# FangjinhuaWang/IterMVS

Hardware: AMD Instinct MI355X
Metric: depth-maps/sec (ref-views/s) at 5-view 640x512, 4 iters (higher is better)
Workload: dtype f32; 1 GPU; BASELINE cfg 2 (= cfg 1 on 1xMI355X): 1 ref + 4 src views, 640x512, 4 GRU iterations, test mode, random-init weights, 1 ref view(s) per step and GPU; views=5, height=512, width=640, batch_per_gpu=1, streams_per_gpu=1, feature_dtype=fp32, launch=one hipGraph per depth map, parallelism=ref-view sharding x1, no collective, projection=device_fp64, conv_arithmetic=bf16x3, side_branch=False

## Files before the change

include/itermvs_hip.h:

```cpp
#ifndef ITERMVS_HIP_H
#define ITERMVS_HIP_H

#include <stdint.h>

#ifdef __cplusplus
extern "C" {
#endif

#if defined(__GNUC__) || defined(__clang__)
#pragma GCC visibility push(default)
#endif

#define ITERMVS_ABI_VERSION 20
#define ITERMVS_MAX_SRC 16
#define ITERMVS_MAX_HYP 8
#define ITERMVS_GROUPS 8
#define ITERMVS_PROB_BINS 256
#define ITERMVS_WINDOW_RADIUS 4

typedef enum itermvs_status {
    ITERMVS_OK = 0,
    ITERMVS_ERR_NULL = -1,
    ITERMVS_ERR_DIMS = -2,
    ITERMVS_ERR_CHANNELS = -3,
// ... 246 lines not shown
    ITERMVS_WALK_PLAIN = 2,
    ITERMVS_WALK_STRIDED_LEAD = 3
} itermvs_walk_kind;

typedef struct itermvs_persistent_plan_t {
    int32_t grid, banded, run, run_extra;
} itermvs_persistent_plan_t;

int itermvs_persistent_plan(int64_t tiles, int32_t resident, int32_t round8, int32_t kind, itermvs_persistent_plan_t* out);
int itermvs_tile_walk_owner(const itermvs_persistent_plan_t* plan, int64_t tiles, int32_t kind, int32_t lead, int32_t* owner, int32_t* order);

int itermvs_corrnet(const float* x, int64_t x_sn, const float* const* weights, const int32_t* seg_end, int32_t n_seg,
                    int32_t M, int32_t H, int32_t W, float* out, int64_t out_sn, float* out2, int64_t out2_sn, void* stream);
int itermvs_corrnet_bf16x3(const float* x, int64_t x_sn, const float* const* weights, const int32_t* seg_end, int32_t n_seg,
                           int32_t M, int32_t H, int32_t W, float* out, int64_t out_sn, float* out2, int64_t out2_sn, void* stream);


int itermvs_stem(const float* x, int64_t x_sn, int32_t M, int32_t H, int32_t W, const float* w0, const float* w1,
                 float* y, float* sc, int64_t out_sn, int32_t out_layout, void* stream);
int itermvs_stem_compose(const float* x, int64_t x_sn, int32_t M, int32_t H, int32_t W, const float* w0, const float* w1,
                         float* y, float* sc, int64_t out_sn, int32_t out_layout, const float* mats, int32_t n_sets, int32_t V, float* proj_out,
                         int32_t* nan_flag, const float* depth_min, const float* depth_max, int32_t Bd, float* inv_min,
                         float* inv_max, void* stream);



int itermvs_fuse_depth(const float* depth_ref, const float* conf_ref, const float* const* depth_src,
                       const float* mats, int32_t S, int32_t H, int32_t W, double geo_pixel_thres,
                       float geo_depth_thres, float photo_thres, int32_t geo_mask_thres, double* depth_avg,
                       uint8_t* photo_mask, uint8_t* geo_mask, uint8_t* final_mask, int32_t* geo_sum,
                       void* stream);

int itermvs_fuse_depth_claim(const float* depth_ref, const float* conf_ref, const float* const* depth_src,
                             const float* mats, int32_t S, int32_t H, int32_t W, double geo_pixel_thres,
                             float geo_depth_thres, float photo_thres, int32_t geo_mask_thres, double* depth_avg,
                             uint8_t* photo_mask, uint8_t* geo_mask, uint8_t* final_mask, int32_t* geo_sum,
                             const uint8_t* claimed_ref, uint8_t* const* claimed_src, void* stream);

int itermvs_fuse_points_workspace_bytes(int32_t H, int32_t W);
int itermvs_fuse_points(const double* depth_avg, const uint8_t* final_mask, const uint8_t* photo_mask,
                        const uint8_t* geo_mask, const float* cam, const uint8_t* rgb, int32_t H, int32_t W,
                        uint8_t* records, int64_t capacity, uint64_t* cursor, int64_t* view_counts, int32_t view,
                        uint32_t* workspace, void* stream);

int itermvs_fuse_points_normals(const double* depth_avg, const uint8_t* final_mask, const uint8_t* photo_mask,
                                const uint8_t* geo_mask, const float* cam, const uint8_t* rgb, int32_t H, int32_t W,
// ... 93 lines not shown
```

itermvs_amd/_lib.py:

```python
from __future__ import annotations

import ctypes as C
import os
from typing import Optional

MAX_SRC = 16
MAX_HYP = 8
GROUPS = 8
F32, F16, BF16 = 0, 1, 2
GT_DTU, GT_BLENDEDMVS = 0, 1
ABI_VERSION = 20

_HERE = os.path.dirname(os.path.abspath(__file__))
LIB_PATH = os.path.join(_HERE, "libitermvs_hip.so")

c_float_p = C.POINTER(C.c_float)


class FMap(C.Structure):
    _fields_ = [("data", C.c_void_p), ("sb", C.c_int64), ("sc", C.c_int64), ("sy", C.c_int64),
                ("sx", C.c_int64), ("C", C.c_int32), ("H", C.c_int32), ("W", C.c_int32), ("dtype", C.c_int32)]


class LevelSrc(C.Structure):
# ... 119 lines not shown
                                      C.c_void_p]),
    "itermvs_conv2d": (C.c_int, [C.POINTER(ConvParams), C.c_void_p]),
    "itermvs_conv2d_plan": (C.c_int, [C.POINTER(ConvParams), C.POINTER(ConvPlan)]),
    "itermvs_persistent_plan": (C.c_int, [C.c_int64, C.c_int32, C.c_int32, C.c_int32, C.POINTER(PersistentPlan)]),
    "itermvs_tile_walk_owner": (C.c_int, [C.POINTER(PersistentPlan), C.c_int64, C.c_int32, C.c_int32, C.c_void_p, C.c_void_p]),
    "itermvs_corrnet": (C.c_int, [C.c_void_p, C.c_int64, C.POINTER(C.c_void_p), C.POINTER(C.c_int32), C.c_int32, C.c_int32, C.c_int32,
                                  C.c_int32, C.c_void_p, C.c_int64, C.c_void_p, C.c_int64, C.c_void_p]),
    "itermvs_corrnet_bf16x3": (C.c_int, [C.c_void_p, C.c_int64, C.POINTER(C.c_void_p), C.POINTER(C.c_int32), C.c_int32, C.c_int32, C.c_int32,
                                  C.c_int32, C.c_void_p, C.c_int64, C.c_void_p, C.c_int64, C.c_void_p]),
    "itermvs_res_chain16": (C.c_int, [C.c_void_p, C.c_int64, C.c_void_p, C.c_int64, C.c_int32, C.c_int32, C.c_int32, C.c_int32,
                                      C.POINTER(C.c_void_p), C.POINTER(C.c_void_p), C.c_void_p, C.c_int64, C.c_void_p]),
    "itermvs_down_conv": (C.c_int, [C.c_void_p, C.c_int64, C.c_int32, C.c_int32, C.c_int32, C.c_int32, C.c_void_p, C.c_void_p, C.c_int32,
                                    C.c_void_p, C.c_int64, C.c_void_p, C.c_int64, C.c_void_p]),
    "itermvs_lateral_conv3x3": (C.c_int, [C.c_void_p, C.c_int64, C.c_int32, C.c_void_p, C.c_int64, C.c_int32, C.c_int32, C.c_int32,
                                          C.c_void_p, C.c_void_p, C.c_void_p, C.c_void_p, C.c_int32, C.c_void_p, C.c_int64, C.c_int32,
                                          C.c_void_p, C.c_void_p]),
    "itermvs_gru_conv": (C.c_int, [C.c_void_p, C.c_int64, C.c_int32, C.c_int32, C.c_int32, C.c_int32, C.c_void_p, C.c_void_p, C.c_void_p,
                                   C.c_int64, C.c_void_p, C.c_int64, C.c_void_p, C.c_int64, C.c_void_p, C.c_int64, C.c_void_p]),
    "itermvs_stem": (C.c_int, [C.c_void_p, C.c_int64, C.c_int32, C.c_int32, C.c_int32, C.c_void_p, C.c_void_p, C.c_void_p, C.c_void_p,
                               C.c_int64, C.c_int32, C.c_void_p]),
    "itermvs_stem_compose": (C.c_int, [C.c_void_p, C.c_int64, C.c_int32, C.c_int32, C.c_int32, C.c_void_p, C.c_void_p, C.c_void_p, C.c_void_p,
                                       C.c_int64, C.c_int32, C.c_void_p, C.c_int32, C.c_int32, C.c_void_p, C.c_void_p, C.c_void_p, C.c_void_p,
                                       C.c_int32, C.c_void_p, C.c_void_p, C.c_void_p]),
    "itermvs_image_pyramid": (C.c_int, [C.c_void_p] + [C.c_int32] * 5 + [C.c_void_p] * 5),
    "itermvs_resize_rgb8": (C.c_int, [C.c_void_p] + [C.c_int32] * 5 + [C.c_void_p, C.c_void_p, C.c_int32, C.c_void_p, C.c_void_p,
                                                                 C.c_int32, C.c_void_p, C.c_void_p]),
    "itermvs_undistort_rgb8": (C.c_int, [C.c_void_p, C.c_int32, C.c_int32, C.c_int32, C.POINTER(C.c_double), C.c_int32] +
                               [C.c_double] * 4 + [C.c_int32, C.c_int32, C.c_void_p, C.c_void_p, C.c_void_p]),
    "itermvs_image_pyramid_jitter": (C.c_int, [C.c_void_p] + [C.c_int32] * 5 + [C.c_void_p] * 7),
    "itermvs_gt_pyramid": (C.c_int, [C.c_void_p] * 3 + [C.c_int32] * 6 + [C.c_void_p] * 9),
    "itermvs_bn_workspace_floats": (C.c_int, [C.c_int32, C.c_int32, C.c_int32]),
    "itermvs_bn_train_forward": (C.c_int, [C.c_void_p, C.c_void_p, C.c_int32, C.c_int32, C.c_int32, C.c_void_p, C.c_void_p,
                                           C.c_float, C.c_float, C.c_int32, C.c_void_p, C.c_void_p, C.c_void_p, C.c_void_p,
                                           C.c_void_p, C.c_void_p]),
    "itermvs_bn_train_backward": (C.c_int, [C.c_void_p, C.c_void_p, C.c_void_p, C.c_int32, C.c_int32, C.c_int32, C.c_void_p,
                                            C.c_void_p, C.c_void_p, C.c_void_p, C.c_int32, C.c_void_p, C.c_void_p, C.c_void_p,
                                            C.c_void_p]),
    "itermvs_profile_enable": (C.c_int, [C.c_int32]),
    "itermvs_profile_set_mask": (C.c_int, [C.c_int32]),
    "itermvs_fuse_depth": (C.c_int, [C.c_void_p, C.c_void_p, C.c_void_p, C.c_void_p, C.c_int32, C.c_int32, C.c_int32, C.c_double,
                                     C.c_float, C.c_float, C.c_int32, C.c_void_p, C.c_void_p, C.c_void_p, C.c_void_p, C.c_void_p,
                                     C.c_void_p]),
    "itermvs_fuse_depth_claim": (C.c_int, [C.c_void_p, C.c_void_p, C.c_void_p, C.c_void_p, C.c_int32, C.c_int32, C.c_int32,
                                           C.c_double, C.c_float, C.c_float, C.c_int32, C.c_void_p, C.c_void_p, C.c_void_p,
                                           C.c_void_p, C.c_void_p, C.c_void_p, C.c_void_p, C.c_void_p]),
    "itermvs_fuse_points_workspace_bytes": (C.c_int, [C.c_int32, C.c_int32]),
# ... 78 lines not shown
```

itermvs_amd/csrc/stem.hip:

```cpp
#include "common.hpp"
#include "compose.hpp"
#include "tile_walk.hpp"
#include <cstdlib>

namespace itermvs {

using f32x4 = __attribute__((ext_vector_type(4))) float;
typedef __attribute__((address_space(4))) float ConstF;

constexpr int kStTW = 32;
constexpr int kStThreads = 256;
constexpr int kStIP = 68;
constexpr int kStFP = 66;

struct StemArgs {
    const float* x;
    const float* w0;
    const float* w1;
    float* y;
    float* sc;
    int64_t x_sn, out_sn;
    int M, H, W, H2, W2, tiles_x, tiles_y;
    int out_c4;
};

using f32x2 = __attribute__((ext_vector_type(2))) float;

template <int kStTH>
struct StemPatch {
    static constexpr int IR = 2 * kStTH + 3, ROWS = 3 * IR, PER = (ROWS + 3) / 4;
    float v[PER], vt[PER];
    unsigned rowok;
    bool c0ok, c1ok;
    __device__ __forceinline__ void fetch(const StemArgs& a, int tile, int wave, int lane) {
        int t = tile;
        const int tx = t % a.tiles_x; t /= a.tiles_x;
        const int ty = t % a.tiles_y;
        const int n = t / a.tiles_y;
        const int iy0 = 2 * ty * kStTH - 2, ix0 = 2 * tx * kStTW - 2;
        const float* __restrict__ xp = a.x + (int64_t)n * a.x_sn;
        const int plane = a.H * a.W;
        const int gx0 = ix0 + lane, gx1 = ix0 + 64 + (lane < 3 ? lane : 2);
        c0ok = gx0 >= 0 && gx0 < a.W;
        c1ok = lane < 3 && gx1 < a.W;
        const int cx0 = min(max(gx0, 0), a.W - 1), cx1 = min(gx1, a.W - 1);
        rowok = 0;
#pragma unroll
        for (int i = 0; i < PER; ++i) {
            const int row = min(wave + 4 * i, ROWS - 1);
            const int ci = row / IR, r = row - ci * IR;
            const int gy = iy0 + r;
            rowok |= (wave + 4 * i < ROWS && gy >= 0 && gy < a.H) ? 1u << i : 0u;
            const float* __restrict__ rp = xp + ci * plane + min(max(gy, 0), a.H - 1) * a.W;
            v[i] = rp[cx0];
            vt[i] = rp[cx1];
        }
    }
    __device__ __forceinline__ void commit(float* __restrict__ IMG, int wave, int lane) const {
#pragma unroll
        for (int i = 0; i < PER; ++i) {
            const int row = wave + 4 * i;
            if (row < ROWS) {
                const bool rok = rowok >> i & 1u;
                IMG[row * kStIP + lane] = rok && c0ok ? v[i] : 0.0f;
                if (lane < 3) IMG[row * kStIP + 64 + lane] = rok && c1ok ? vt[i] : 0.0f;
            }
        }
    }
};

template <int kStTH>
__global__ __launch_bounds__(kStThreads) void stem_kernel(StemArgs a, int tiles, int n_comp, ComposeArgs comp) {
    if ((int)blockIdx.x < n_comp) {
        compose_proj_body(comp, (int)blockIdx.x * kStThreads + (int)threadIdx.x);
        return;
    }
    const TileWalk walk = tile_walk_strided(tiles, blockIdx.x, gridDim.x, n_comp, (int)gridDim.x - n_comp >= 8);
    const int tile0 = walk.w, tstep = walk.wstep, tend = walk.wend;

    constexpr int kStIR = 2 * kStTH + 3, kStFR = 2 * kStTH + 1;
    constexpr int kStFPL = kStFR * kStFP + 1;
    static_assert(kStFPL % 2 == 1, "f0 plane stride must be odd");
    __shared__ float IMG[3 * kStIR * kStIP];
    __shared__ float F0[8 * kStFPL];
    const int tid = threadIdx.x, lane = tid & 63;
    const int wave = __builtin_amdgcn_readfirstlane(tid >> 6);
    const int q = lane >> 4, l16 = lane & 15;

    StemPatch<kStTH> patch;
    if (tile0 < tend) patch.fetch(a, tile0, wave, lane);

    float aw[36];
#pragma unroll
    for (int i = 0; i < 18; ++i) {
        aw[2 * i] = a.w1[(i * 4 + q) * 32 + l16];
        aw[2 * i + 1] = a.w1[(i * 4 + q) * 32 + 16 + l16];
    }
    const float* __restrict__ bias = a.w1 + 9 * 2 * 4 * 32;
    float bv[2][4];
#pragma unroll
    for (int mb = 0; mb < 2; ++mb)
#pragma unroll
        for (int r = 0; r < 4; ++r) bv[mb][r] = bias[mb * 16 + q * 4 + r];
    const int oplane = a.H2 * a.W2;

#pragma unroll 1
    for (int tile = tile0; tile < tend; tile += tstep) {
        int t = tile;
        const int tx = t % a.tiles_x; t /= a.tiles_x;
        const int ty = t % a.tiles_y;
        const int n = t / a.tiles_y;
        const int oy0 = ty * kStTH, ox0 = tx * kStTW;
        const int iy0 = 2 * oy0 - 2, ix0 = 2 * ox0 - 2;

        patch.commit(IMG, wave, lane);
        __syncthreads();
        if (tile + tstep < tend) patch.fetch(a, tile + tstep, wave, lane);

        constexpr int ITEMS = kStFR * 64 + kStFR, ROUNDS = (ITEMS + kStThreads - 1) / kStThreads;
#pragma unroll 1
        for (int it = 0; it < ROUNDS; ++it) {
            int opaque = 0;
            asm volatile("" : "+s"(opaque));
            const ConstF* w0 = (const ConstF*)(uintptr_t)a.w0 + __builtin_amdgcn_readfirstlane(opaque);
            const int rr = wave + 4 * it;
            const bool tail = rr >= kStFR;
            const int r = tail ? lane : rr, c = tail ? 64 : lane;
            if (tail && (rr > kStFR || lane >= kStFR)) continue;
            float v[27];
            const float* __restrict__ ip = IMG + r * kStIP + c;
#pragma unroll
            for (int ci = 0; ci < 3; ++ci)
#pragma unroll
                for (int ky = 0; ky < 3; ++ky)
#pragma unroll
                    for (int kx = 0; kx < 3; ++kx) v[(ci * 3 + ky) * 3 + kx] = ip[(ci * kStIR + ky) * kStIP + kx];
            const int gy = iy0 + 1 + r, gx = ix0 + 1 + c;
            const bool inside = gy >= 0 && gy < a.H && gx >= 0 && gx < a.W;
            f32x2 acc[4];
#pragma unroll
            for (int c2 = 0; c2 < 4; ++c2) acc[c2] = f32x2{w0[216 + 2 * c2], w0[217 + 2 * c2]};
#pragma unroll
            for (int k = 0; k < 27; ++k)
#pragma unroll
                for (int c2 = 0; c2 < 4; ++c2)
                    acc[c2] = __builtin_elementwise_fma(f32x2{w0[k * 8 + 2 * c2], w0[k * 8 + 2 * c2 + 1]}, f32x2{v[k], v[k]}, acc[c2]);
            float* __restrict__ fp = F0 + r * kStFP + c;
#pragma unroll
            for (int co = 0; co < 8; ++co) fp[co * kStFPL] = inside ? fmaxf(acc[co >> 1][co & 1], 0.0f) : 0.0f;
        }
        __syncthreads();

#pragma unroll
        for (int gi = 0; gi < kStTH / 2; ++gi) {
            const int g = wave + 4 * gi;
            const int oy = g >> 1, oxl = (g & 1) * 16 + l16;
            f32x4 acc[2];
#pragma unroll
            for (int mb = 0; mb < 2; ++mb) acc[mb] = f32x4{bv[mb][0], bv[mb][1], bv[mb][2], bv[mb][3]};
            const float* __restrict__ bp = F0 + q * kStFPL + 2 * oy * kStFP + 2 * oxl;
#pragma unroll
            for (int tap = 0; tap < 9; ++tap) {
                const int ky = tap / 3, kx = tap - ky * 3;
#pragma unroll
                for (int ks = 0; ks < 2; ++ks) {
                    const float b = bp[ks * 4 * kStFPL + ky * kStFP + kx];
                    acc[0] = __builtin_amdgcn_mfma_f32_16x16x4f32(aw[(tap * 2 + ks) * 2], b, acc[0], 0, 0, 0);
                    acc[1] = __builtin_amdgcn_mfma_f32_16x16x4f32(aw[(tap * 2 + ks) * 2 + 1], b, acc[1], 0, 0, 0);
                }
            }
            const int gy = oy0 + oy, gx = ox0 + oxl;
            if (gy < a.H2 && gx < a.W2) {
                if (a.out_c4) {
                    const int64_t o = (int64_t)n * a.out_sn + ((int64_t)q * oplane + gy * a.W2 + gx) * 4;
                    *reinterpret_cast<f32x4*>(a.y + o) =
                        f32x4{fmaxf(acc[0][0], 0.0f), fmaxf(acc[0][1], 0.0f), fmaxf(acc[0][2], 0.0f), fmaxf(acc[0][3], 0.0f)};
                    *reinterpret_cast<f32x4*>(a.sc + o) = acc[1];
                } else {
                    const int64_t o = (int64_t)n * a.out_sn + (int64_t)(q * 4) * oplane + gy * a.W2 + gx;
                    float* __restrict__ yo = a.y + o;
                    float* __restrict__ so = a.sc + o;
#pragma unroll
                    for (int r = 0; r < 4; ++r) {
                        yo[r * oplane] = fmaxf(acc[0][r], 0.0f);
                        so[r * oplane] = acc[1][r];
                    }
                }
            }
        }
    }
}

}

static int launch_stem(const float* x, int64_t x_sn, int32_t M, int32_t H, int32_t W, const float* w0, const float* w1,
                       float* y, float* sc, int64_t out_sn, int32_t out_layout, const itermvs::ComposeArgs* comp, void* stream) {
    using namespace itermvs;
    if (!x || !w0 || !w1 || !y || !sc) return ITERMVS_ERR_NULL;
    if (M < 0 || H < 1 || W < 1) return ITERMVS_ERR_DIMS;
    if (out_layout != 0 && out_layout != 1) return ITERMVS_ERR_LAYOUT;
    if (out_layout == 1 && (((uintptr_t)y | (uintptr_t)sc) % 16 || out_sn % 4)) return ITERMVS_ERR_ALIGN;
    ComposeArgs c{};
    int n_comp = 0;
    if (comp) {
        c = *comp;
        int ct = c.n_sets * (c.V - 1);
        if (c.inv_min && c.B > ct) ct = c.B;
        n_comp = (ct + kStThreads - 1) / kStThreads;
    }
    if (M == 0 && n_comp == 0) return ITERMVS_OK;
    StemArgs a;
    a.x = x; a.w0 = w0; a.w1 = w1; a.y = y; a.sc = sc;
    a.x_sn = x_sn; a.out_sn = out_sn; a.out_c4 = out_layout;
    a.M = M; a.H = H; a.W = W;
    a.H2 = (H - 1) / 2 + 1; a.W2 = (W - 1) / 2 + 1;
    static const int th = [] { const char* e = itermvs_tuning_env("ITERMVS_STEM_TH"); return e && atoi(e) == 4 ? 4 : 8; }();
    a.tiles_x = (a.W2 + kStTW - 1) / kStTW; a.tiles_y = (a.H2 + th - 1) / th;
    const int64_t tiles = (int64_t)M * a.tiles_x * a.tiles_y;
    static const int wg_per_cu = [] { const char* e = itermvs_tuning_env("ITERMVS_STEM_WGS"); return e ? atoi(e) : 0; }();
    PersistentPlan plan = {};
    if (tiles != 0) {
        const int rc = persistent_plan_cus(tiles, wg_per_cu > 0 ? wg_per_cu : (th == 4 ? 4 : 3), false, ITERMVS_WALK_STRIDED_LEAD, &plan);
        if (rc != ITERMVS_OK) return rc;
    }
    const unsigned grid = (unsigned)plan.grid + (unsigned)n_comp;
    if (th == 4) hipLaunchKernelGGL(stem_kernel<4>, dim3(grid), dim3(kStThreads), 0, (hipStream_t)stream, a, (int)tiles, n_comp, c);
    else hipLaunchKernelGGL(stem_kernel<8>, dim3(grid), dim3(kStThreads), 0, (hipStream_t)stream, a, (int)tiles, n_comp, c);
    return itermvs_launch_status();
}

extern "C" int itermvs_stem(const float* x, int64_t x_sn, int32_t M, int32_t H, int32_t W, const float* w0, const float* w1,
                            float* y, float* sc, int64_t out_sn, int32_t out_layout, void* stream) {
    return launch_stem(x, x_sn, M, H, W, w0, w1, y, sc, out_sn, out_layout, nullptr, stream);
}

extern "C" int itermvs_stem_compose(const float* x, int64_t x_sn, int32_t M, int32_t H, int32_t W, const float* w0, const float* w1,
                                    float* y, float* sc, int64_t out_sn, int32_t out_layout, const float* mats, int32_t n_sets, int32_t V,
                                    float* proj_out, int32_t* nan_flag, const float* depth_min, const float* depth_max, int32_t Bd,
                                    float* inv_min, float* inv_max, void* stream) {
    ITERMVS_RETURN_IF(!mats || !proj_out, ITERMVS_ERR_NULL);
    ITERMVS_RETURN_IF(inv_min && (!depth_min || !depth_max || !inv_max || Bd < 1), ITERMVS_ERR_NULL);
    ITERMVS_RETURN_IF(n_sets < 1, ITERMVS_ERR_DIMS);
    ITERMVS_RETURN_IF(V < 2 || V - 1 > ITERMVS_MAX_SRC, ITERMVS_ERR_VIEWS);
    const itermvs::ComposeArgs c{mats, proj_out, nan_flag, depth_min, depth_max, inv_min, inv_max, n_sets, V, Bd};
    return launch_stem(x, x_sn, M, H, W, w0, w1, y, sc, out_sn, out_layout, &c, stream);
}
```

itermvs_amd/engine.py:

```python
from __future__ import annotations

import gc
import itertools
import weakref
from typing import Dict, List, Mapping, Tuple

import torch

from . import ops

Tensor = torch.Tensor

INIT_SAMPLES = 32
HIDDEN = 32
_INTERVALS = {1: (-2.0, -2.0 / 3, 2.0 / 3, 2.0), 2: (-8.0, -8.0 / 3, 8.0 / 3, 8.0), 3: (-32.0, 32.0)}


def sample_offsets() -> Dict[int, Tuple[float, ...]]:
    out = {}
    for l, vals in _INTERVALS.items():
        t = torch.tensor(vals, dtype=torch.float32) * (1.0 / 256)
        out[l] = tuple(float(v) for v in t)
    return out

# ... 43 lines not shown
        self.side_branch = side_branch
        self._side = None
        self.profile_iterations = None
        self.profile_init = True
        self.pk: Dict[str, object] = {}
        self._pack_weights()

    def _pack_weights(self) -> None:
        w, pk = self.w, self.pk
        pack = lambda wt: ops.pack_conv_weight(wt) if (wt.shape[1] <= 4 or wt.shape[0] == 1) and wt.shape[2] == 3 else ops.MfmaWeight(wt, split3=self.split3)
        for n, (wt, _) in self.cbr.items():
            pk["feature_net." + n] = pack(wt)
        for k, v in w.items():
            if not k.endswith("weight") or v.dim() != 4 or ".bn." in k or k.startswith("feature_net.") and ".conv." in k:
                continue
            if k.endswith("conv3.weight") or k.endswith("conv4.weight"):
                pk[k] = ops.MfmaWeight(v, transposed=True)
            else:
                pk[k] = pack(v)
        pv = "iter_mvs.evaluation.pixel_view_weight.conv.1."
        cf = "iter_mvs.update.confidence_head.2."
        self.conf_dot = torch.cat([w[cf + "weight"].reshape(-1), w[cf + "bias"].reshape(-1)]).float().contiguous()
        self.pvw_dot = torch.cat([w[pv + "weight"].reshape(-1), w[pv + "bias"].reshape(-1)]).float().contiguous()
        self.stem_w = ops.pack_stem_weights(*self.cbr["conv1."], *self.cbr["layer1.0.conv1."], *self.cbr["layer1.0.downsample."])
        self.corrnet_w = {l: ops.pack_corrnet_weights(w, f"iter_mvs.evaluation.corr_conv1.{l - 1}.", split3=self.split3) for l in (1, 2, 3)}
        dh = "iter_mvs.update.depth_head."
        self.head_w1, self.head_w2 = ops.pack_head_weights(w[dh + "2.weight"], w[dh + "4.weight"])
        if self.split3:
            self.head_w2_fused = ops.pack_head_w2_split3(w[dh + "4.weight"])
            self.head_w0_fused = ops.pack_head_w0_split3(w[dh + "0.weight"])
        else:
            self.head_w2_fused = self.head_w2
            self.head_w0_fused = None
        self.pk_zr = ops.MfmaWeight(self.w_zr, split3=False)
        self.gru_coop = self.split3
        if self.gru_coop:
            g = "iter_mvs.update.gru."
            self.gru_zr = ops.pack_gru_conv_split3(self.w_zr)
            self.gru_q = ops.pack_gru_conv_split3(w[g + "convq.weight"])
            self.gru_bq = w[g + "convq.bias"].contiguous()
        hi, up = "iter_mvs.update.hidden_init_head.", "iter_mvs.upsample."
        self.pk_hi0, self.pk_up0 = ops.MfmaWeight(w[hi + "0.weight"], split3=False), ops.MfmaWeight(w[up + "0.weight"], split3=False)
        self.hi1, self.hi1_bias = ops.pack_conv1x1_operand(w[hi + "2.weight"], w[hi + "2.bias"])
        self.up1, _ = ops.pack_conv1x1_operand(w[up + "2.weight"])
        if self.split3:
            self.pk_hi0, self.hi1, self.hi1_bias = ops.pack_conv3x3_conv1x1_split3(w[hi + "0.weight"], w[hi + "2.weight"], w[hi + "2.bias"])
            self.pk_up0, self.up1, _ = ops.pack_conv3x3_conv1x1_split3(w[up + "0.weight"], w[up + "2.weight"])
# ... 27 lines not shown
            y = ops.conv2d(x, wt, bias, stride=2, act="relu", split=(c, "none", sc))
        return self._cbr(y, name + "conv2.", 1, "relu", add=sc)

    def feature_net(self, x: Tensor, compose=None, out: Tuple[Tensor, Tensor, Tensor, Tensor] = None) -> Dict[int, Tensor]:
        p = "feature_net."
        m, _, hh, ww = x.shape
        dev = x.device
        if out is not None:
            o1, o2, o3, self.o2_planar = out
            want = [((m, 16, hh // 2, ww // 2), self.feature_dtype), ((m, 32, hh // 4, ww // 4), self.feature_dtype),
                    ((m, 48, hh // 8, ww // 8), self.feature_dtype)]
            for t, (shape, dt) in zip((o1, o2, o3), want):
                if tuple(t.shape) != shape or t.dtype != dt or not t.is_contiguous(memory_format=torch.channels_last):
                    raise RuntimeError(f"feature_net: out level must be a dense channels-last {dt} tensor {shape}")
            p2 = self.o2_planar
            if tuple(p2.shape) != (m, 32, hh // 4, ww // 4) or p2.dtype != torch.float32 or not p2.is_contiguous():
                raise RuntimeError(f"feature_net: the planar level-2 map must be a contiguous float32 {(m, 32, hh // 4, ww // 4)}")
        else:
            cl = lambda c, s: torch.empty((m, c, hh // s, ww // s), device=dev, dtype=self.feature_dtype,
                                          memory_format=torch.channels_last)
            o1, o2, o3 = cl(16, 2), cl(32, 4), cl(48, 8)
            self.o2_planar = torch.empty((m, 32, hh // 4, ww // 4), device=dev)
        if compose is not None:
            y, sc, *self.composed = ops.stem(x, *self.stem_w, compose=compose, quads=self.split3)
        else:
            y, sc = ops.stem(x, *self.stem_w, quads=self.split3)
        if self.split3:
            names = ("layer1.0.conv2.", "layer1.1.conv1.", "layer1.1.conv2.")
            f1 = ops.res_chain16(y, sc, [self.pk[p + k] for k in names], [self.cbr[k][1] for k in names], quads=True)
        else:
            f1 = self._res(self._cbr(y, "layer1.0.conv2.", 1, "relu", add=sc), "layer1.1.", 1)
        f2 = self._res(self._res(f1, "layer2.0.", 2), "layer2.1.", 1)
        f3 = self._res(self._res(f2, "layer3.0.", 2), "layer3.1.", 1)
        self._conv(f3, p + "output3.", bias=True, channels_last_out=True, out=o3)
        mid = self._conv(f2, p + "inner2.", bias=True, ksize=1, pad=0, add=f3, add_up2=True)
        self._conv(mid, p + "output2.", bias=True, channels_last_out=True, out=o2, out2=self.o2_planar)
        if self.split3:
            ops.lateral_conv3x3(f1, mid, self.pk[p + "inner1.weight"], self.w[p + "inner1.bias"], self.pk[p + "output1.weight"],
                                self.w[p + "output1.bias"], out=o1, channels_last_out=True)
        else:
            mid = self._conv(f1, p + "inner1.", bias=True, ksize=1, pad=0, add=mid, add_up2=True)
            self._conv(mid, p + "output1.", bias=True, channels_last_out=True, out=o1)
        return {1: o1, 2: o2, 3: o3}

    def corr_nets(self, x: Tensor, levels, seg_end=(), out: Tensor = None, out2: Tensor = None) -> Tensor:
        return ops.corrnet(x, [self.corrnet_w[l] for l in levels], seg_end, out=out, out2=out2)

    def depth_head(self, hidden: Tensor) -> Tensor:
        p = "iter_mvs.update.depth_head."
# ... 541 lines not shown
```

itermvs_amd/ops.py:

```python
from __future__ import annotations

import contextlib
import ctypes as C
import os
from typing import Dict, List, NamedTuple, Optional, Sequence, Tuple

import numpy as np
import torch

from . import _lib
from ._lib import MAX_HYP, MAX_SRC, ConvParams, CorrInitParams, CorrIterParams, FMap, LevelSlots, LevelSrc, TapParams, check

Tensor = torch.Tensor


def _stream() -> int:
    return torch.cuda.current_stream().cuda_stream


def _dev(t: Tensor, name: str) -> Tensor:
    if not isinstance(t, torch.Tensor) or not t.is_cuda:
        raise RuntimeError(f"{name}: expected a CUDA/ROCm tensor - the IterMVS HIP engine has no CPU path")
    if t.dtype != torch.float32:
        raise RuntimeError(f"{name}: expected float32, got {t.dtype}")
# ... 1499 lines not shown
        for v in range(6):
            for term in (h, m_):
                ops_a.append(torch.stack([term[2 * v], term[2 * v + 1], term[2 * v], term[2 * v + 1]]))
        for v in range(6):
            ops_a.append(torch.stack([l[2 * v], l[2 * v + 1], h[2 * v], h[2 * v + 1]]))
        first = torch.stack(ops_a).contiguous().view(torch.int16).reshape(-1).view(torch.float32)
    else:
        first = _mfma_operand_order(two.reshape(12, 8, 16), 16)
    if split3:
        as_floats = lambda wt: MfmaWeight(wt, split3=True).tile3.contiguous().view(torch.int16).reshape(-1).view(torch.float32)
        mid = [as_floats(w[prefix + "conv2.conv.weight"].float()),
               as_floats(w[prefix + "conv3.weight"].float().permute(1, 0, 2, 3)),
               as_floats(w[prefix + "conv4.weight"].float().permute(1, 0, 2, 3))]
    else:
        mid = [conv("conv2.conv.weight", 32), dconv("conv3.weight", 16), dconv("conv4.weight", 16)]
    parts = [first, conv("conv1.conv.weight", 16)] + mid + [
             w[prefix + "conv5.weight"].float().permute(1, 2, 3, 0).reshape(-1), w[prefix + "conv5.bias"].float().reshape(-1)]
    flat = torch.cat(parts + [torch.zeros(7, device=parts[0].device)])
    assert flat.numel() == (CORRNET_WEIGHT_FLOATS_SPLIT3 if split3 else CORRNET_WEIGHT_FLOATS)
    return flat.contiguous()


STEM_W0_FLOATS, STEM_W1_FLOATS = 224, 2336


def pack_stem_weights(w0: Tensor, b0: Tensor, w1: Tensor, b1: Tensor, wd: Tensor, bd: Tensor) -> Tuple[Tensor, Tensor]:
    if tuple(w0.shape) != (8, 3, 3, 3) or tuple(w1.shape) != (16, 8, 3, 3) or tuple(wd.shape) != (16, 8, 3, 3):
        raise RuntimeError("pack_stem_weights: expects conv1 [8,3,3,3] and two stride-2 layers [16,8,3,3]")
    p0 = torch.cat([w0.float().permute(1, 2, 3, 0).reshape(-1), b0.float().reshape(-1)]).contiguous()
    wc = torch.cat([w1, wd]).float()
    p1 = torch.cat([_mfma_operand_order(wc.permute(2, 3, 1, 0).reshape(9, 8, 32), 32), b1.float().reshape(-1),
                    bd.float().reshape(-1)]).contiguous()
    assert p0.numel() == STEM_W0_FLOATS and p1.numel() == STEM_W1_FLOATS
    return p0, p1


def stem(x: Tensor, w0: Tensor, w1: Tensor, compose=None, quads: bool = False):
    ptr, x_sn = _planes(x, "stem input")
    m, c, h, w = x.shape
    if c != 3:
        raise RuntimeError("stem: expects [M,3,H,W]")
    if w0.numel() != STEM_W0_FLOATS or w1.numel() != STEM_W1_FLOATS:
        raise RuntimeError("stem: weights must come from pack_stem_weights")
    h2, w2 = (h - 1) // 2 + 1, (w - 1) // 2 + 1
    y = torch.empty((m, 4, h2, w2, 4) if quads else (m, 16, h2, w2), device=x.device, dtype=torch.float32)
    sc = torch.empty_like(y)
    if compose is not None:
        mats, nan_flag, depth_range = compose
        mats = _dev(mats, "mats").contiguous()
        n, v = mats.shape[0], mats.shape[1]
        proj = torch.empty((n, v - 1, 12), device=mats.device, dtype=torch.float32)
        dmin, dmax = (_dev(t, "depth range").contiguous() for t in depth_range)
        imin, imax = torch.empty_like(dmin), torch.empty_like(dmax)
        check(_lib.load().itermvs_stem_compose(ptr, x_sn, m, h, w, _dev(w0, "stem weights").data_ptr(), _dev(w1, "stem weights").data_ptr(),
                                               y.data_ptr(), sc.data_ptr(), 16 * h2 * w2, int(quads), mats.data_ptr(), n, v, proj.data_ptr(),
                                               _ptr(nan_flag), dmin.data_ptr(), dmax.data_ptr(), dmin.numel(), imin.data_ptr(),
                                               imax.data_ptr(), _stream()), "itermvs_stem_compose")
        return y, sc, proj, imin, imax
    check(_lib.load().itermvs_stem(ptr, x_sn, m, h, w, _dev(w0, "stem weights").data_ptr(), _dev(w1, "stem weights").data_ptr(),
                             y.data_ptr(), sc.data_ptr(), 16 * h2 * w2, int(quads), _stream()), "itermvs_stem")
    return y, sc


def res_chain16(y1: Tensor, shortcut: Tensor, weights: Sequence["MfmaWeight"], biases: Sequence[Optional[Tensor]],
                out: Optional[Tensor] = None, quads: bool = False) -> Tensor:
    if quads:
        for t, name in ((y1, "res_chain16 input"), (shortcut, "res_chain16 shortcut")):
            _dev(t, name)
            if t.dim() != 5 or t.shape[1] != 4 or t.shape[4] != 4 or not t.is_contiguous():
                raise RuntimeError(f"{name}: quads layout is a contiguous [N,4,H,W,4] tensor")
        n, _, h, w, _ = y1.shape
        if tuple(shortcut.shape) != tuple(y1.shape):
            raise RuntimeError("res_chain16: input and shortcut differ in shape")
        ptr, y_sn, sp, s_sn = y1.data_ptr(), 16 * h * w, shortcut.data_ptr(), 16 * h * w
    else:
        ptr, y_sn = _planes(y1, "res_chain16 input")
        sp, s_sn = _planes(shortcut, "res_chain16 shortcut")
        n, c, h, w = y1.shape
        if c != 16 or tuple(shortcut.shape) != (n, c, h, w):
            raise RuntimeError("res_chain16: expects two [N,16,H,W] tensors")
    if len(weights) != 3 or len(biases) != 3:
        raise RuntimeError("res_chain16: three layers")
    for wt in weights:
# ... 256 lines not shown
```

Before: 1159 depth-maps/s.

## Port stem stride-2 conv to bf16x3 MFMA with split-plane LDS layout

Adds a bf16x3 variant of the stem kernel. It splits the conv1 output into high, middle and low bf16 planes stored in a parity-decomposed shared-memory layout, then runs the stride-2 16x8x3x3 convolutions with 16x16x32 bf16 MFMAs in place of fp32 16x16x4 MFMAs. Weights are pre-split and packed by a new host-side path. When split3 is on, the tile height defaults to 4 and residency to 3 workgroups per CU, and LDS is now dynamic. The aim is to cut MFMA instruction count in the stem, at the cost of more split arithmetic and LDS, and slightly different rounding.

```diff
diff --git a/include/itermvs_hip.h b/include/itermvs_hip.h
--- a/include/itermvs_hip.h
+++ b/include/itermvs_hip.h
@@ -292,6 +292,12 @@
                          float* y, float* sc, int64_t out_sn, int32_t out_layout, const float* mats, int32_t n_sets, int32_t V, float* proj_out,
                          int32_t* nan_flag, const float* depth_min, const float* depth_max, int32_t Bd, float* inv_min,
                          float* inv_max, void* stream);
+int itermvs_stem_bf16x3(const float* x, int64_t x_sn, int32_t M, int32_t H, int32_t W, const float* w0, const void* w1_split,
+                        float* y, float* sc, int64_t out_sn, int32_t out_layout, void* stream);
+int itermvs_stem_compose_bf16x3(const float* x, int64_t x_sn, int32_t M, int32_t H, int32_t W, const float* w0, const void* w1_split,
+                                float* y, float* sc, int64_t out_sn, int32_t out_layout, const float* mats, int32_t n_sets, int32_t V,
+                                float* proj_out, int32_t* nan_flag, const float* depth_min, const float* depth_max, int32_t Bd,
+                                float* inv_min, float* inv_max, void* stream);
 
 
 
diff --git a/itermvs_amd/_lib.py b/itermvs_amd/_lib.py
--- a/itermvs_amd/_lib.py
+++ b/itermvs_amd/_lib.py
@@ -165,6 +165,11 @@
     "itermvs_stem_compose": (C.c_int, [C.c_void_p, C.c_int64, C.c_int32, C.c_int32, C.c_int32, C.c_void_p, C.c_void_p, C.c_void_p, C.c_void_p,
                                        C.c_int64, C.c_int32, C.c_void_p, C.c_int32, C.c_int32, C.c_void_p, C.c_void_p, C.c_void_p, C.c_void_p,
                                        C.c_int32, C.c_void_p, C.c_void_p, C.c_void_p]),
+    "itermvs_stem_bf16x3": (C.c_int, [C.c_void_p, C.c_int64, C.c_int32, C.c_int32, C.c_int32, C.c_void_p, C.c_void_p, C.c_void_p, C.c_void_p,
+                                      C.c_int64, C.c_int32, C.c_void_p]),
+    "itermvs_stem_compose_bf16x3": (C.c_int, [C.c_void_p, C.c_int64, C.c_int32, C.c_int32, C.c_int32, C.c_void_p, C.c_void_p, C.c_void_p,
+                                              C.c_void_p, C.c_int64, C.c_int32, C.c_void_p, C.c_int32, C.c_int32, C.c_void_p, C.c_void_p,
+                                              C.c_void_p, C.c_void_p, C.c_int32, C.c_void_p, C.c_void_p, C.c_void_p]),
     "itermvs_image_pyramid": (C.c_int, [C.c_void_p] + [C.c_int32] * 5 + [C.c_void_p] * 5),
     "itermvs_resize_rgb8": (C.c_int, [C.c_void_p] + [C.c_int32] * 5 + [C.c_void_p, C.c_void_p, C.c_int32, C.c_void_p, C.c_void_p,
                                                                  C.c_int32, C.c_void_p, C.c_void_p]),
diff --git a/itermvs_amd/csrc/stem.hip b/itermvs_amd/csrc/stem.hip
--- a/itermvs_amd/csrc/stem.hip
+++ b/itermvs_amd/csrc/stem.hip
@@ -25,6 +25,17 @@
 };
 
 using f32x2 = __attribute__((ext_vector_type(2))) float;
+
+template <int kStTH>
+struct StemGeom3 {
+    static constexpr int CW = 33;
+    static constexpr int CP = ((kStTH + 1) * CW - 4 + 7) / 8 * 8 + 4;
+    static constexpr int CSB = CP * 16, PLB = 4 * CSB;
+    static constexpr int F0B = 3 * PLB;
+    static constexpr int LDS = F0B + 3 * (2 * kStTH + 3) * kStIP * 4;
+    static_assert(PLB % 256 == 0 && CSB % 128 == 64 && LDS <= 80 * 1024, "f0 image geometry");
+};
+constexpr int kStW1SBytes = 2 * 8 * 64 * 16;
 
 template <int kStTH>
 struct StemPatch {
@@ -69,7 +80,7 @@
     }
 };
 
-template <int kStTH>
+template <int kStTH, bool S3>
 __global__ __launch_bounds__(kStThreads) void stem_kernel(StemArgs a, int tiles, int n_comp, ComposeArgs comp) {
     if ((int)blockIdx.x < n_comp) {
         compose_proj_body(comp, (int)blockIdx.x * kStThreads + (int)threadIdx.x);
@@ -81,8 +92,10 @@
     constexpr int kStIR = 2 * kStTH + 3, kStFR = 2 * kStTH + 1;
     constexpr int kStFPL = kStFR * kStFP + 1;
     static_assert(kStFPL % 2 == 1, "f0 plane stride must be odd");
-    __shared__ float IMG[3 * kStIR * kStIP];
-    __shared__ float F0[8 * kStFPL];
+    using G3 = StemGeom3<kStTH>;
+    extern __shared__ __attribute__((aligned(16))) char dsm[];
+    float* const IMG = reinterpret_cast<float*>(dsm + (S3 ? G3::F0B : 0));
+    float* const F0 = IMG + 3 * kStIR * kStIP;
     const int tid = threadIdx.x, lane = tid & 63;
     const int wave = __builtin_amdgcn_readfirstlane(tid >> 6);
     const int q = lane >> 4, l16 = lane & 15;
@@ -90,19 +103,39 @@
     StemPatch<kStTH> patch;
     if (tile0 < tend) patch.fetch(a, tile0, wave, lane);
 
-    float aw[36];
-#pragma unroll
-    for (int i = 0; i < 18; ++i) {
-        aw[2 * i] = a.w1[(i * 4 + q) * 32 + l16];
-        aw[2 * i + 1] = a.w1[(i * 4 + q) * 32 + 16 + l16];
-    }
-    const float* __restrict__ bias = a.w1 + 9 * 2 * 4 * 32;
+    float aw[S3 ? 1 : 36];
+    bf8 aw3[S3 ? 2 : 1][S3 ? 8 : 1];
+    if constexpr (S3) {
+        const bf8* __restrict__ src = reinterpret_cast<const bf8*>(a.w1);
+#pragma unroll
+        for (int mb = 0; mb < 2; ++mb)
+#pragma unroll
+            for (int o = 0; o < 8; ++o) aw3[mb][o] = src[(mb * 8 + o) * 64 + lane];
+    } else {
+#pragma unroll
+        for (int i = 0; i < 18; ++i) {
+            aw[2 * i] = a.w1[(i * 4 + q) * 32 + l16];
+            aw[2 * i + 1] = a.w1[(i * 4 + q) * 32 + 16 + l16];
+        }
+    }
+    const float* __restrict__ bias = S3 ? a.w1 + kStW1SBytes / 4 : a.w1 + 9 * 2 * 4 * 32;
     float bv[2][4];
 #pragma unroll
     for (int mb = 0; mb < 2; ++mb)
 #pragma unroll
         for (int r = 0; r < 4; ++r) bv[mb][r] = bias[mb * 16 + q * 4 + r];
     const int oplane = a.H2 * a.W2;
+    int bo3[4] = {0, 0, 0, 0};
+    if constexpr (S3) {
+#pragma unroll
+        for (int ks = 0; ks < 2; ++ks) {
+            const int tap = 4 * ks + q, ky = tap / 3, kx = tap - ky * 3;
+            bo3[ks] = ((ky & 1) * 2 + (kx & 1)) * G3::CSB + ((ky >> 1) * G3::CW + (kx >> 1)) * 16;
+        }
+        const int t8 = (G3::CW + 1) * 16;
+        bo3[2] = (q == 1 ? 1 : q == 2 ? 2 : 0) * G3::PLB + t8;
+        bo3[3] = (q == 0 ? 1 : 0) * G3::PLB + t8;
+    }
 
 #pragma unroll 1
     for (int tile = tile0; tile < tend; tile += tstep) {
@@ -145,9 +178,23 @@
 #pragma unroll
                 for (int c2 = 0; c2 < 4; ++c2)
                     acc[c2] = __builtin_elementwise_fma(f32x2{w0[k * 8 + 2 * c2], w0[k * 8 + 2 * c2 + 1]}, f32x2{v[k], v[k]}, acc[c2]);
-            float* __restrict__ fp = F0 + r * kStFP + c;
-#pragma unroll
-            for (int co = 0; co < 8; ++co) fp[co * kStFPL] = inside ? fmaxf(acc[co >> 1][co & 1], 0.0f) : 0.0f;
+            if constexpr (S3) {
+                u32x4 Hh, Mm, Ll;
+#pragma unroll
+                for (int c2 = 0; c2 < 4; ++c2) {
+                    uint32_t h, m, l;
+                    split_pair(inside ? fmaxf(acc[c2][0], 0.0f) : 0.0f, inside ? fmaxf(acc[c2][1], 0.0f) : 0.0f, h, m, l);
+                    Hh[c2] = h; Mm[c2] = m; Ll[c2] = l;
+                }
+                char* __restrict__ d = dsm + ((r & 1) * 2 + (c & 1)) * G3::CSB + ((r >> 1) * G3::CW + (c >> 1)) * 16;
+                *reinterpret_cast<u32x4*>(d) = Hh;
+                *reinterpret_cast<u32x4*>(d + G3::PLB) = Mm;
+                *reinterpret_cast<u32x4*>(d + 2 * G3::PLB) = Ll;
+            } else {
+                float* __restrict__ fp = F0 + r * kStFP + c;
+#pragma unroll
+                for (int co = 0; co < 8; ++co) fp[co * kStFPL] = inside ? fmaxf(acc[co >> 1][co & 1], 0.0f) : 0.0f;
+            }
         }
         __syncthreads();
 
@@ -158,15 +205,40 @@
             f32x4 acc[2];
 #pragma unroll
             for (int mb = 0; mb < 2; ++mb) acc[mb] = f32x4{bv[mb][0], bv[mb][1], bv[mb][2], bv[mb][3]};
-            const float* __restrict__ bp = F0 + q * kStFPL + 2 * oy * kStFP + 2 * oxl;
-#pragma unroll
-            for (int tap = 0; tap < 9; ++tap) {
-                const int ky = tap / 3, kx = tap - ky * 3;
-#pragma unroll
-                for (int ks = 0; ks < 2; ++ks) {
-                    const float b = bp[ks * 4 * kStFPL + ky * kStFP + kx];
-                    acc[0] = __builtin_amdgcn_mfma_f32_16x16x4f32(aw[(tap * 2 + ks) * 2], b, acc[0], 0, 0, 0);
-                    acc[1] = __builtin_amdgcn_mfma_f32_16x16x4f32(aw[(tap * 2 + ks) * 2 + 1], b, acc[1], 0, 0, 0);
+            if constexpr (S3) {
+                const char* __restrict__ bp = dsm + (oy * G3::CW + oxl) * 16;
+                bf8 b[2][3], bx, by;
+#pragma unroll
+                for (int ks = 0; ks < 2; ++ks)
+#pragma unroll
+                    for (int t = 0; t < 3; ++t) b[ks][t] = *reinterpret_cast<const bf8*>(bp + t * G3::PLB + bo3[ks]);
+                bx = *reinterpret_cast<const bf8*>(bp + bo3[2]);
+                by = *reinterpret_cast<const bf8*>(bp + bo3[3]);
+                constexpr int kW[6] = {2, 0, 1, 1, 0, 0}, kX[6] = {0, 2, 1, 0, 1, 0};
+#pragma unroll
+                for (int half = 0; half < 2; ++half) {
+#pragma unroll
+                    for (int ks = 0; ks < 2; ++ks)
+#pragma unroll
+                        for (int p = 3 * half; p < 3 * half + 3; ++p)
+#pragma unroll
+                            for (int mb = 0; mb < 2; ++mb)
+                                acc[mb] = __builtin_amdgcn_mfma_f32_16x16x32_bf16(aw3[mb][ks * 3 + kW[p]], b[ks][kX[p]], acc[mb], 0, 0, 0);
+#pragma unroll
+                    for (int mb = 0; mb < 2; ++mb)
+                        acc[mb] = __builtin_amdgcn_mfma_f32_16x16x32_bf16(aw3[mb][half ? 6 : 7], half ? bx : by, acc[mb], 0, 0, 0);
+                }
+            } else {
+                const float* __restrict__ bp = F0 + q * kStFPL + 2 * oy * kStFP + 2 * oxl;
+#pragma unroll
+                for (int tap = 0; tap < 9; ++tap) {
+                    const int ky = tap / 3, kx = tap - ky * 3;
+#pragma unroll
+                    for (int ks = 0; ks < 2; ++ks) {
+                        const float b = bp[ks * 4 * kStFPL + ky * kStFP + kx];
+                        acc[0] = __builtin_amdgcn_mfma_f32_16x16x4f32(aw[(tap * 2 + ks) * 2], b, acc[0], 0, 0, 0);
+                        acc[1] = __builtin_amdgcn_mfma_f32_16x16x4f32(aw[(tap * 2 + ks) * 2 + 1], b, acc[1], 0, 0, 0);
+                    }
                 }
             }
             const int gy = oy0 + oy, gx = ox0 + oxl;
@@ -193,13 +265,25 @@
 
 }
 
-static int launch_stem(const float* x, int64_t x_sn, int32_t M, int32_t H, int32_t W, const float* w0, const float* w1,
+namespace itermvs {
+template <int TH, bool S3>
+constexpr int stem_lds_bytes() {
+    return S3 ? StemGeom3<TH>::LDS : (3 * (2 * TH + 3) * kStIP + 8 * ((2 * TH + 1) * kStFP + 1)) * 4;
+}
+template <int TH, bool S3>
+static int launch_stem_kernel(unsigned grid, hipStream_t stream, const StemArgs& a, int tiles, int n_comp, const ComposeArgs& c) {
+    return launch_fused<stem_kernel<TH, S3>, stem_lds_bytes<TH, S3>()>(dim3(grid), kStThreads, stream, false, a, tiles, n_comp, c);
+}
+}
+
+static int launch_stem(const float* x, int64_t x_sn, int32_t M, int32_t H, int32_t W, const float* w0, const float* w1, bool split3,
                        float* y, float* sc, int64_t out_sn, int32_t out_layout, const itermvs::ComposeArgs* comp, void* stream) {
     using namespace itermvs;
     if (!x || !w0 || !w1 || !y || !sc) return ITERMVS_ERR_NULL;
     if (M < 0 || H < 1 || W < 1) return ITERMVS_ERR_DIMS;
     if (out_layout != 0 && out_layout != 1) return ITERMVS_ERR_LAYOUT;
     if (out_layout == 1 && (((uintptr_t)y | (uintptr_t)sc) % 16 || out_sn % 4)) return ITERMVS_ERR_ALIGN;
+    if (split3 && (uintptr_t)w1 % 16) return ITERMVS_ERR_ALIGN;
     ComposeArgs c{};
     int n_comp = 0;
     if (comp) {
@@ -214,34 +298,59 @@
     a.x_sn = x_sn; a.out_sn = out_sn; a.out_c4 = out_layout;
     a.M = M; a.H = H; a.W = W;
     a.H2 = (H - 1) / 2 + 1; a.W2 = (W - 1) / 2 + 1;
-    static const int th = [] { const char* e = itermvs_tuning_env("ITERMVS_STEM_TH"); return e && atoi(e) == 4 ? 4 : 8; }();
+    static const int th_env = [] { const char* e = itermvs_tuning_env("ITERMVS_STEM_TH"); return e ? atoi(e) : 0; }();
+    const int th = th_env == 4 || th_env == 8 ? th_env : split3 ? 4 : 8;
     a.tiles_x = (a.W2 + kStTW - 1) / kStTW; a.tiles_y = (a.H2 + th - 1) / th;
     const int64_t tiles = (int64_t)M * a.tiles_x * a.tiles_y;
     static const int wg_per_cu = [] { const char* e = itermvs_tuning_env("ITERMVS_STEM_WGS"); return e ? atoi(e) : 0; }();
+    const int resident = wg_per_cu > 0 ? wg_per_cu : split3 ? (th == 4 ? 3 : 2) : (th == 4 ? 4 : 3);
     PersistentPlan plan = {};
     if (tiles != 0) {
-        const int rc = persistent_plan_cus(tiles, wg_per_cu > 0 ? wg_per_cu : (th == 4 ? 4 : 3), false, ITERMVS_WALK_STRIDED_LEAD, &plan);
+        const int rc = persistent_plan_cus(tiles, resident, false, ITERMVS_WALK_STRIDED_LEAD, &plan);
         if (rc != ITERMVS_OK) return rc;
     }
     const unsigned grid = (unsigned)plan.grid + (unsigned)n_comp;
-    if (th == 4) hipLaunchKernelGGL(stem_kernel<4>, dim3(grid), dim3(kStThreads), 0, (hipStream_t)stream, a, (int)tiles, n_comp, c);
-    else hipLaunchKernelGGL(stem_kernel<8>, dim3(grid), dim3(kStThreads), 0, (hipStream_t)stream, a, (int)tiles, n_comp, c);
-    return itermvs_launch_status();
+    const hipStream_t s = (hipStream_t)stream;
+    if (split3) return th == 4 ? launch_stem_kernel<4, true>(grid, s, a, (int)tiles, n_comp, c) : launch_stem_kernel<8, true>(grid, s, a, (int)tiles, n_comp, c);
+    return th == 4 ? launch_stem_kernel<4, false>(grid, s, a, (int)tiles, n_comp, c) : launch_stem_kernel<8, false>(grid, s, a, (int)tiles, n_comp, c);
+}
+
+static int check_compose(const float* mats, int32_t n_sets, int32_t V, const float* proj_out, const float* depth_min, const float* depth_max,
+                         int32_t Bd, const float* inv_min, const float* inv_max) {
+    ITERMVS_RETURN_IF(!mats || !proj_out, ITERMVS_ERR_NULL);
+    ITERMVS_RETURN_IF(inv_min && (!depth_min || !depth_max || !inv_max || Bd < 1), ITERMVS_ERR_NULL);
+    ITERMVS_RETURN_IF(n_sets < 1, ITERMVS_ERR_DIMS);
+    ITERMVS_RETURN_IF(V < 2 || V - 1 > ITERMVS_MAX_SRC, ITERMVS_ERR_VIEWS);
+    return ITERMVS_OK;
 }
 
 extern "C" int itermvs_stem(const float* x, int64_t x_sn, int32_t M, int32_t H, int32_t W, const float* w0, const float* w1,
                             float* y, float* sc, int64_t out_sn, int32_t out_layout, void* stream) {
-    return launch_stem(x, x_sn, M, H, W, w0, w1, y, sc, out_sn, out_layout, nullptr, stream);
+    return launch_stem(x, x_sn, M, H, W, w0, w1, false, y, sc, out_sn, out_layout, nullptr, stream);
 }
 
 extern "C" int itermvs_stem_compose(const float* x, int64_t x_sn, int32_t M, int32_t H, int32_t W, const float* w0, const float* w1,
                                     float* y, float* sc, int64_t out_sn, int32_t out_layout, const float* mats, int32_t n_sets, int32_t V,
                                     float* proj_out, int32_t* nan_flag, const float* depth_min, const float* depth_max, int32_t Bd,
                                     float* inv_min, float* inv_max, void* stream) {
-    ITERMVS_RETURN_IF(!mats || !proj_out, ITERMVS_ERR_NULL);
-    ITERMVS_RETURN_IF(inv_min && (!depth_min || !depth_max || !inv_max || Bd < 1), ITERMVS_ERR_NULL);
-    ITERMVS_RETURN_IF(n_sets < 1, ITERMVS_ERR_DIMS);
-    ITERMVS_RETURN_IF(V < 2 || V - 1 > ITERMVS_MAX_SRC, ITERMVS_ERR_VIEWS);
+    const int rc = check_compose(mats, n_sets, V, proj_out, depth_min, depth_max, Bd, inv_min, inv_max);
+    ITERMVS_RETURN_IF(rc != ITERMVS_OK, rc);
     const itermvs::ComposeArgs c{mats, proj_out, nan_flag, depth_min, depth_max, inv_min, inv_max, n_sets, V, Bd};
-    return launch_stem(x, x_sn, M, H, W, w0, w1, y, sc, out_sn, out_layout, &c, stream);
-}
+    return launch_stem(x, x_sn, M, H, W, w0, w1, false, y, sc, out_sn, out_layout, &c, stream);
+}
+
+extern "C" int itermvs_stem_bf16x3(const float* x, int64_t x_sn, int32_t M, int32_t H, int32_t W, const float* w0, const void* w1_split,
+                                   float* y, float* sc, int64_t out_sn, int32_t out_layout, void* stream) {
+    return launch_stem(x, x_sn, M, H, W, w0, static_cast<const float*>(w1_split), true, y, sc, out_sn, out_layout, nullptr, stream);
+}
+
+extern "C" int itermvs_stem_compose_bf16x3(const float* x, int64_t x_sn, int32_t M, int32_t H, int32_t W, const float* w0,
+                                           const void* w1_split, float* y, float* sc, int64_t out_sn, int32_t out_layout,
+                                           const float* mats, int32_t n_sets, int32_t V, float* proj_out, int32_t* nan_flag,
+                                           const float* depth_min, const float* depth_max, int32_t Bd, float* inv_min, float* inv_max,
+                                           void* stream) {
+    const int rc = check_compose(mats, n_sets, V, proj_out, depth_min, depth_max, Bd, inv_min, inv_max);
+    ITERMVS_RETURN_IF(rc != ITERMVS_OK, rc);
+    const itermvs::ComposeArgs c{mats, proj_out, nan_flag, depth_min, depth_max, inv_min, inv_max, n_sets, V, Bd};
+    return launch_stem(x, x_sn, M, H, W, w0, static_cast<const float*>(w1_split), true, y, sc, out_sn, out_layout, &c, stream);
+}
diff --git a/itermvs_amd/engine.py b/itermvs_amd/engine.py
--- a/itermvs_amd/engine.py
+++ b/itermvs_amd/engine.py
@@ -89,7 +89,8 @@
         cf = "iter_mvs.update.confidence_head.2."
         self.conf_dot = torch.cat([w[cf + "weight"].reshape(-1), w[cf + "bias"].reshape(-1)]).float().contiguous()
         self.pvw_dot = torch.cat([w[pv + "weight"].reshape(-1), w[pv + "bias"].reshape(-1)]).float().contiguous()
-        self.stem_w = ops.pack_stem_weights(*self.cbr["conv1."], *self.cbr["layer1.0.conv1."], *self.cbr["layer1.0.downsample."])
+        self.stem_w = ops.pack_stem_weights(*self.cbr["conv1."], *self.cbr["layer1.0.conv1."], *self.cbr["layer1.0.downsample."],
+                                            split3=self.split3)
         self.corrnet_w = {l: ops.pack_corrnet_weights(w, f"iter_mvs.evaluation.corr_conv1.{l - 1}.", split3=self.split3) for l in (1, 2, 3)}
         dh = "iter_mvs.update.depth_head."
         self.head_w1, self.head_w2 = ops.pack_head_weights(w[dh + "2.weight"], w[dh + "4.weight"])
@@ -163,9 +164,9 @@
             o1, o2, o3 = cl(16, 2), cl(32, 4), cl(48, 8)
             self.o2_planar = torch.empty((m, 32, hh // 4, ww // 4), device=dev)
         if compose is not None:
-            y, sc, *self.composed = ops.stem(x, *self.stem_w, compose=compose, quads=self.split3)
-        else:
-            y, sc = ops.stem(x, *self.stem_w, quads=self.split3)
+            y, sc, *self.composed = ops.stem(x, *self.stem_w, compose=compose, quads=self.split3, split3=self.split3)
+        else:
+            y, sc = ops.stem(x, *self.stem_w, quads=self.split3, split3=self.split3)
         if self.split3:
             names = ("layer1.0.conv2.", "layer1.1.conv1.", "layer1.1.conv2.")
             f1 = ops.res_chain16(y, sc, [self.pk[p + k] for k in names], [self.cbr[k][1] for k in names], quads=True)
diff --git a/itermvs_amd/ops.py b/itermvs_amd/ops.py
--- a/itermvs_amd/ops.py
+++ b/itermvs_amd/ops.py
@@ -1545,29 +1545,46 @@
 
 
 STEM_W0_FLOATS, STEM_W1_FLOATS = 224, 2336
-
-
-def pack_stem_weights(w0: Tensor, b0: Tensor, w1: Tensor, b1: Tensor, wd: Tensor, bd: Tensor) -> Tuple[Tensor, Tensor]:
+STEM_W1_SPLIT_WORDS = 2 * 8 * 64 * 4 + 32
+
+
+def pack_stem_weights(w0: Tensor, b0: Tensor, w1: Tensor, b1: Tensor, wd: Tensor, bd: Tensor, split3: bool = False) -> Tuple[Tensor, Tensor]:
     if tuple(w0.shape) != (8, 3, 3, 3) or tuple(w1.shape) != (16, 8, 3, 3) or tuple(wd.shape) != (16, 8, 3, 3):
         raise RuntimeError("pack_stem_weights: expects conv1 [8,3,3,3] and two stride-2 layers [16,8,3,3]")
     p0 = torch.cat([w0.float().permute(1, 2, 3, 0).reshape(-1), b0.float().reshape(-1)]).contiguous()
     wc = torch.cat([w1, wd]).float()
+    assert p0.numel() == STEM_W0_FLOATS
+    if split3:
+        terms = torch.stack(split_bf16x3(wc.reshape(2, 16, 8, 9).permute(0, 3, 1, 2).contiguous()))
+        zero = torch.zeros_like(terms[0, :, 8])
+        t8 = lambda *ts: torch.stack([zero if t is None else terms[t, :, 8] for t in ts], 1)
+        operands = [terms[t, :, 4 * ks:4 * ks + 4] for ks in (0, 1) for t in (0, 1, 2)] + [t8(0, 0, 0, 1), t8(1, 2, None, None)]
+        words = torch.stack(operands, 1).contiguous().view(torch.int32).reshape(-1)
+        bias = torch.cat([b1.float().reshape(-1), bd.float().reshape(-1)]).contiguous().view(torch.int32)
+        p1 = torch.cat([words, bias]).contiguous()
+        assert p1.numel() == STEM_W1_SPLIT_WORDS
+        return p0, p1
     p1 = torch.cat([_mfma_operand_order(wc.permute(2, 3, 1, 0).reshape(9, 8, 32), 32), b1.float().reshape(-1),
                     bd.float().reshape(-1)]).contiguous()
-    assert p0.numel() == STEM_W0_FLOATS and p1.numel() == STEM_W1_FLOATS
+    assert p1.numel() == STEM_W1_FLOATS
     return p0, p1
 
 
-def stem(x: Tensor, w0: Tensor, w1: Tensor, compose=None, quads: bool = False):
+def stem(x: Tensor, w0: Tensor, w1: Tensor, compose=None, quads: bool = False, split3: Optional[bool] = None):
     ptr, x_sn = _planes(x, "stem input")
     m, c, h, w = x.shape
     if c != 3:
         raise RuntimeError("stem: expects [M,3,H,W]")
-    if w0.numel() != STEM_W0_FLOATS or w1.numel() != STEM_W1_FLOATS:
-        raise RuntimeError("stem: weights must come from pack_stem_weights")
+    if split3 is None:
+        split3 = w1.dtype == torch.int32
+    if w0.numel() != STEM_W0_FLOATS or w0.dtype != torch.float32 or (w1.dtype, w1.numel()) != (
+            (torch.int32, STEM_W1_SPLIT_WORDS) if split3 else (torch.float32, STEM_W1_FLOATS)):
+        raise RuntimeError("stem: weights must come from pack_stem_weights (split3=True for the bf16x3 form)")
+    suffix = "_bf16x3" if split3 else ""
     h2, w2 = (h - 1) // 2 + 1, (w - 1) // 2 + 1
     y = torch.empty((m, 4, h2, w2, 4) if quads else (m, 16, h2, w2), device=x.device, dtype=torch.float32)
     sc = torch.empty_like(y)
+    w0p, w1p = _dev(w0, "stem weights").data_ptr(), _dev(w1.view(torch.float32), "stem weights").data_ptr()
     if compose is not None:
         mats, nan_flag, depth_range = compose
         mats = _dev(mats, "mats").contiguous()
@@ -1575,13 +1592,13 @@
         proj = torch.empty((n, v - 1, 12), device=mats.device, dtype=torch.float32)
         dmin, dmax = (_dev(t, "depth range").contiguous() for t in depth_range)
         imin, imax = torch.empty_like(dmin), torch.empty_like(dmax)
-        check(_lib.load().itermvs_stem_compose(ptr, x_sn, m, h, w, _dev(w0, "stem weights").data_ptr(), _dev(w1, "stem weights").data_ptr(),
-                                               y.data_ptr(), sc.data_ptr(), 16 * h2 * w2, int(quads), mats.data_ptr(), n, v, proj.data_ptr(),
-                                               _ptr(nan_flag), dmin.data_ptr(), dmax.data_ptr(), dmin.numel(), imin.data_ptr(),
-                                               imax.data_ptr(), _stream()), "itermvs_stem_compose")
+        name = "itermvs_stem_compose" + suffix
+        check(getattr(_lib.load(), name)(ptr, x_sn, m, h, w, w0p, w1p, y.data_ptr(), sc.data_ptr(), 16 * h2 * w2, int(quads), mats.data_ptr(),
+                                         n, v, proj.data_ptr(), _ptr(nan_flag), dmin.data_ptr(), dmax.data_ptr(), dmin.numel(),
+                                         imin.data_ptr(), imax.data_ptr(), _stream()), name)
         return y, sc, proj, imin, imax
-    check(_lib.load().itermvs_stem(ptr, x_sn, m, h, w, _dev(w0, "stem weights").data_ptr(), _dev(w1, "stem weights").data_ptr(),
-                             y.data_ptr(), sc.data_ptr(), 16 * h2 * w2, int(quads), _stream()), "itermvs_stem")
+    name = "itermvs_stem" + suffix
+    check(getattr(_lib.load(), name)(ptr, x_sn, m, h, w, w0p, w1p, y.data_ptr(), sc.data_ptr(), 16 * h2 * w2, int(quads), _stream()), name)
     return y, sc
 
 
```

Measured after the change: 1162 depth-maps/s, median of 6. No clear change (+0.3%).
